# centreborelli/sat-bundleadjust

Measured on AMD Instinct MI355X. Metric: LM iters/sec at 200 cams x 1M pts x 10M obs (affine, R+T), higher is better.
Workload: dtype f64; 1 GPU; C4: 200 cams x 1000000 pts x 9998866 obs, affine, correction R+T, 1 fixed camera, seed 1; obs_per_rank0=9998866

## Files before the change

sat-bundleadjust_amd/csrc/satba_capi.hip:

```cpp
#include <hip/hip_runtime.h>

#include <algorithm>
#include <atomic>
#include <chrono>
#include <cmath>
#include <cstdarg>
#include <cstdio>
#include <cstdlib>
#include <cstring>
#include <new>
#include <string>
#include <thread>
#include <vector>

#include "../../include/satba.h"
#include "satba_chol.h"
#include "satba_kernels.h"
#include "satba_layout.h"
#include "satba_lm.h"
#include "satba_lmdev.h"
#include "satba_outliers.h"
#include "satba_triangulate.h"
#include "satba_tracks.h"
#include "satba_ftracks.h"
// ... 48 lines not shown
        if (e_ != hipSuccess) return fail(SATBA_E_HIP, "%s: %s (%s:%d)", #expr, hipGetErrorString(e_), __FILE__, __LINE__); \
    } while (0)

constexpr int RED_SLOTS = 8, RED_MAX_GRID = 2048, RED_MAX_NV = 4;
struct SchurItems { int2* items = nullptr; SchurItem* desc = nullptr; int n_blocks = 0; };
static_assert(sizeof(SchurItemKey) == sizeof(int2) && offsetof(SchurItemKey, pair) == offsetof(int2, x) && offsetof(SchurItemKey, chunk) == offsetof(int2, y), "uploaded as int2");

struct satba_problem {
    int model = 0, M = 0, N = 0, NP = 0, c_p = 0, n_cam_fix = 0, n_pts_fix = 0, rank = 0, world = 1, f32 = 0, device = 0;
    long long K = 0, n_total = 0;
    int n_c = 0, n = 0, hdr = 0;
    int loss = 0;
    int camc_lds = 0, rpc_lds = 0;
    int cam_sums_lds = 1;
    int lin_rep_shift = 0;
    int deterministic = 0;
    int split_env = -1;
    double *d_fx = nullptr, *d_bbox = nullptr, *d_fxcost = nullptr, *d_fxcost_new = nullptr, *d_fxcost0 = nullptr;
    int *d_fxflag = nullptr, *d_fxe = nullptr;
    bool fxcost_valid = false, fxcost_new_valid = false, fxcost0_valid = false;
    double w_max = 1.0, n_max_cam = 1.0, fx_shrink = 1.0;
    int fx_fallbacks = 0;
    bool scales_by_tail = false;
    bool prep_fused = false;
    struct LmDev* d_lm = nullptr;
    struct LmSummary* h_lm = nullptr;
    struct LmSummary* h_lm_dev = nullptr;
    long long lm_ticks_queued = 0;
    hipStream_t own_stream = nullptr;
    double f_scale = 1.0, lead = 1.0;
    hipStream_t stream = nullptr;
    Layout L;
    int unit_weights = 0;
    double *d_cam_static = nullptr, *d_rpc = nullptr;
    double *d_x = nullptr, *d_xnew = nullptr, *d_camc = nullptr, *d_camc_new = nullptr;
    double *d_scale_inv = nullptr, *d_g = nullptr, *d_gh = nullptr, *d_gn = nullptr, *d_q1 = nullptr, *d_wv = nullptr;
    double *d_U = nullptr, *d_gc = nullptr, *d_V = nullptr, *d_PV = nullptr, *d_dc = nullptr, *d_dch = nullptr;
    double2 *d_f = nullptr, *d_ftmp = nullptr;
    bool f_valid = false;
    bool prof_lin = false;
    std::vector<hipEvent_t> prof_ev;
    size_t prof_used = 0;
    double* d_Jpm = nullptr;
    double *d_part = nullptr, *d_part3 = nullptr, *d_pair_part = nullptr;
    SchurItems items_chunked;
    SchurItems items_merged;
// ... 205 lines not shown
    if (unit_run(p))
        SATBA_DISPATCH(p, hipLaunchKernelGGL((k_residual<MODEL, NP, CL, RL, true, false>), dim3(grid), dim3(RES_THREADS), lds, p->stream, a, f, p->red(RB_RES), cost, t));
    else
        SATBA_DISPATCH(p, hipLaunchKernelGGL((k_residual<MODEL, NP, CL, RL, false, false>), dim3(grid), dim3(RES_THREADS), lds, p->stream, a, f, p->red(RB_RES), cost, t));
    HIP_TRY(hipGetLastError());
    return 0;
}

static int launch_trial(satba_problem* p, const PhaseCtx& c, double c0, double c1, const double* v0, const double* v1) {
    if (c.decide1a_in_trial) {
        hipLaunchKernelGGL(k_lm_decide1a_trial_cams, dim3(1), dim3(256), 0, p->stream, p->d_lm, p->d_xb, p->model, p->M, p->NP, p->c_p, p->d_x, v0, v1,
                           p->d_scale_inv, p->d_cam_static, p->d_xnew, p->d_camc_new, p->d_xb, (int)p->hdr);
    } else
    hipLaunchKernelGGL(k_trial_cams, dim3((std::max(p->M, (int)p->hdr) + 63) / 64), dim3(64), 0, p->stream, p->model, p->M, p->NP, p->c_p, p->d_x, v0, v1,
                       p->d_scale_inv, c0, c1, p->d_cam_static, p->d_xnew, p->d_camc_new, p->d_xb, (int)p->hdr, c.coef_dev, c.gate);
    HIP_TRY(hipGetLastError());
    ObsArgs a = obs_args(p, true, c.gate);
    a.sh = slice_split(p);
    a.rev = slice_rev(3);
    const int grid = slice_grid(p, RES_THREADS / 64, 2, a.sh);
    const size_t lds = table_bytes(p);
    TrialArgs t{p->d_x, v0, v1, p->d_scale_inv, p->d_xnew, c0, c1, p->lead, p->d_xb + SATBA_HDR_STEP_SQ, p->d_xb + SATBA_HDR_X_SQ, p->d_fxcost_new, c.coef_dev};
    if (c.decide2_in_trial) { t.lm_st = p->d_lm; t.lm_sum = p->h_lm_dev; }
    p->fxcost_new_valid = true;
    double* cost = p->d_xb + SATBA_HDR_COST_NEW;
    if (unit_run(p))
        SATBA_DISPATCH(p, hipLaunchKernelGGL((k_residual<MODEL, NP, CL, RL, true, true>), dim3(grid), dim3(RES_THREADS), lds, p->stream, a, (double2*)nullptr, p->red(RB_RES), cost, t));
    else
        SATBA_DISPATCH(p, hipLaunchKernelGGL((k_residual<MODEL, NP, CL, RL, false, true>), dim3(grid), dim3(RES_THREADS), lds, p->stream, a, (double2*)nullptr, p->red(RB_RES), cost, t));
    HIP_TRY(hipGetLastError());
    return 0;
}

static int lin_variant(const satba_problem* p) {
    if (p->loss == 0) return (p->unit_weights && p->model != RPC) ? 0 : 1;
    return p->loss == SATBA_LOSS_SOFT_L1 ? 2 : 3;
}

template <int MODEL, int NP, bool CL, bool RL>
static int launch_lin(satba_problem* p, const ObsArgs& a) {
    double* gpv = p->d_g + p->n_c;
    double* cost = p->d_xb + SATBA_HDR_COST;
    double* gmax = p->d_xb + SATBA_HDR_FIXED + p->rank;
    const size_t lds = lin_lds(p);
    const RedBuf rb = p->red(RB_LIN);
    constexpr bool BIGL = MODEL == RPC || NP > 6;
// ... 23 lines not shown
    TRY(raise_lds_limit(k_linearize<MODEL, NP, false, CL, RL, false, false, true>, lds));
    TRY(raise_lds_limit(k_linearize<MODEL, NP, false, CL, RL, false, false, false>, lds));
    TRY(raise_lds_limit(k_linearize<MODEL, NP, true, CL, RL, false, false, true>, lds));
    TRY(raise_lds_limit(k_linearize<MODEL, NP, true, CL, RL, false, false, false>, lds));
    TRY(raise_lds_limit(k_linearize<MODEL, NP, true, CL, RL, true, false, true>, lds));
    TRY(raise_lds_limit(k_linearize<MODEL, NP, true, CL, RL, true, false, false>, lds));
    if constexpr (MODEL != RPC) {
        TRY(raise_lds_limit(k_linearize<MODEL, NP, false, CL, RL, false, true, true>, lds));
        TRY(raise_lds_limit(k_linearize<MODEL, NP, false, CL, RL, false, true, false>, lds));
    }
    TRY(raise_lds_limit(k_residual<MODEL, NP, CL, RL, true, false>, table_bytes(p)));
    TRY(raise_lds_limit(k_residual<MODEL, NP, CL, RL, false, false>, table_bytes(p)));
    TRY(raise_lds_limit(k_residual<MODEL, NP, CL, RL, true, true>, table_bytes(p)));
    TRY(raise_lds_limit(k_residual<MODEL, NP, CL, RL, false, true>, table_bytes(p)));
    const size_t dirb = p->dir_global ? 0 : dir_table_bytes(p);
    const size_t t = std::max(table_bytes(p), dirb);
    TRY(raise_lds_limit(k_jvp<MODEL, NP, 1, CL, RL, true>, t));
    TRY(raise_lds_limit(k_jvp<MODEL, NP, 1, CL, RL, false>, t));
    TRY(raise_lds_limit(k_jvp<MODEL, NP, 2, CL, RL, false>, std::max(t, 2 * dirb)));
    TRY(raise_lds_limit(k_backsub<MODEL, NP, CL, RL>, t));
    return 0;
}

static int launch_linearize_kernel(satba_problem* p, const PhaseCtx& c) {
    ObsArgs a = obs_args(p, false, c.gate);
    a.sh = slice_split(p);
    a.rev = slice_rev(0);
    if (c.fuse_prep >= 0) {
        a.prep_scale = p->d_scale_inv; a.prep_gh = p->d_gh; a.prep_ghs = p->d_q1;
        a.prep_first = c.fuse_prep; a.prep_first_dev = c.first_dev;
    }
    const bool prof = p->prof_lin && p->prof_used + 2 <= 2 * 4096;
    if (prof) {
        while (p->prof_ev.size() < p->prof_used + 2) {
            hipEvent_t e;
            HIP_TRY(hipEventCreate(&e));
            p->prof_ev.push_back(e);
        }
        HIP_TRY(hipEventRecord(p->prof_ev[p->prof_used], p->stream));
    }
    SATBA_DISPATCH(p, TRY((launch_lin<MODEL, NP, CL, RL>(p, a))));
    if (prof) {
        HIP_TRY(hipEventRecord(p->prof_ev[p->prof_used + 1], p->stream));
        p->prof_used += 2;
    }
    return 0;
}

static int launch_cam_sums(satba_problem* p, const int* gate, double* U, double* gc) {
    ObsArgs a = obs_args(p, false, gate);
    CamMajor cm = cam_major(p);
    SATBA_DISPATCH(p, hipLaunchKernelGGL((k_cam_sums<MODEL, NP>), dim3(p->M, p->cm_chunks), dim3(LINC_THREADS), 0, p->stream, a, cm, p->d_f, p->d_part3));
// ... 8 lines not shown
struct SchurRoute;
int schur_items_build(satba_problem* p, SchurTable kind, SchurItems* t, long long dg_weight);
int schur_item_tables(satba_problem* p);
template <int MODEL, int NP> int launch_schur(satba_problem* p, const FrontCtx& f, const SchurRoute& r, const ObsArgs& a, double* S, double* rhs);
}
static int launch_schur_kernel(satba_problem* p, const int* gate, const FrontCtx& f, const SchurRoute& r) {
    ObsArgs a = obs_args(p, false, gate);
    double* S = p->payload();
    double* rhs = S + (size_t)p->n_c * p->n_c;
    SATBA_DISPATCH(p, TRY((launch_schur<MODEL, NP>(p, f, r, a, S, rhs))));
    return 0;
}

static int launch_backsub_kernel(satba_problem* p, const int* gate) {
    ObsArgs a = obs_args(p, false, gate);
    a.sh = slice_split(p);
    a.rev = slice_rev(1);
    const int grid = slice_grid(p, BS_THREADS / 64, 2, a.sh);
    const size_t lds = p->model == AFFINE ? dir_table_bytes(p) : table_bytes(p);
    if (p->dir_global) {
        SATBA_DISPATCH(p, if constexpr (MODEL == AFFINE) {
            hipLaunchKernelGGL((k_affine_dir_tab<NP>), dim3(1), dim3(1024), 0, p->stream, a, p->d_dc, (const double*)nullptr, (const double*)nullptr);
            hipLaunchKernelGGL((k_backsub<MODEL, NP, CL, RL, true>), dim3(grid), dim3(BS_THREADS), 0, p->stream, a, p->d_dc, p->d_dch, p->lead,
                               p->d_V, p->d_lam_used, p->d_g, p->d_scale_inv, p->d_gh, p->d_gn, p->red(RB_BS), p->d_xb);
        });
    } else
    SATBA_DISPATCH(p, hipLaunchKernelGGL((k_backsub<MODEL, NP, CL, RL>), dim3(grid), dim3(BS_THREADS), lds, p->stream, a, p->d_dc, p->d_dch, p->lead,
                                         p->d_V, p->d_lam_used, p->d_g, p->d_scale_inv, p->d_gh, p->d_gn, p->red(RB_BS), p->d_xb));
    HIP_TRY(hipGetLastError());
    return 0;
}

static int launch_jvp(satba_problem* p, const int* gate, int nv, const double* q1, const double* q2, double* out, bool pre = false) {
    ObsArgs a = obs_args(p, false, gate);
    a.sh = slice_split(p);
    a.rev = slice_rev(2);
    const int grid = slice_grid(p, JVP_THREADS / 64, 2, a.sh);
    const RedBuf rb = p->red(RB_JVP);
    if (p->dir_global && (nv == 2 || pre)) {
        SATBA_DISPATCH(p, if constexpr (MODEL == AFFINE) {
            hipLaunchKernelGGL((k_affine_dir_tab<NP>), dim3(1), dim3(1024), 0, p->stream, a, q1, nv == 2 ? q2 : nullptr, nv == 2 ? p->d_scale_inv : nullptr);
            if (nv == 1) hipLaunchKernelGGL((k_jvp<MODEL, NP, 1, CL, RL, true, true>), dim3(grid), dim3(JVP_THREADS), 0, p->stream, a, q1, q2, p->d_scale_inv, rb, out);
            else hipLaunchKernelGGL((k_jvp<MODEL, NP, 2, CL, RL, false, true>), dim3(grid), dim3(JVP_THREADS), 0, p->stream, a, q1, q2, p->d_scale_inv, rb, out);
        });
    } else if (nv == 1 && pre) {
        const size_t lds = p->model == AFFINE ? dir_table_bytes(p) : table_bytes(p);
        SATBA_DISPATCH(p, hipLaunchKernelGGL((k_jvp<MODEL, NP, 1, CL, RL, true>), dim3(grid), dim3(JVP_THREADS), lds, p->stream, a, q1, q2, p->d_scale_inv, rb, out));
    } else if (nv == 1) {
        SATBA_DISPATCH(p, hipLaunchKernelGGL((k_jvp<MODEL, NP, 1, CL, RL, false>), dim3(grid), dim3(JVP_THREADS), table_bytes(p), p->stream, a, q1, q2,
                                             p->d_scale_inv, rb, out));
    } else {
        const size_t lds = p->model == AFFINE ? std::max(table_bytes(p), 2 * dir_table_bytes(p)) : table_bytes(p);
        SATBA_DISPATCH(p, hipLaunchKernelGGL((k_jvp<MODEL, NP, 2, CL, RL, false>), dim3(grid), dim3(JVP_THREADS), lds, p->stream, a, q1, q2,
                                             p->d_scale_inv, rb, out));
    }
    HIP_TRY(hipGetLastError());
    return 0;
}

static int dense_solve(satba_problem* p, const int* gate, double* S, double* b, bool cleared = false, bool* unscaled = nullptr) {
    TrsvTail tail;
    tail.dc = p->d_dc; tail.scale_inv = p->d_scale_inv; tail.hdr = p->d_xb; tail.hdr_len = (int)p->hdr; tail.fail = p->d_fail; tail.lead = p->lead;
    tail.keep = p->d_keep; tail.keep_at = SATBA_HDR_KEEP; tail.keep_len = SATBA_KEEP_LEN;
    const bool done = cholesky_solve(S, p->n_c, b, p->d_fail, p->d_fail + 1, p->stream, p->chol, p->d_dinv, cleared, gate, nullptr,
                                     unscaled ? &tail : nullptr);
    if (unscaled) *unscaled = done;
    HIP_TRY(hipGetLastError());
    return 0;
}

__global__ void k_lambda(const double* __restrict__ hdr, double Delta, double lam_floor, double* __restrict__ keep, const double* __restrict__ Delta_dev,
                         const double* __restrict__ lam_force, const int* gate) {
    SATBA_GATE(gate);
    if (Delta_dev) Delta = *Delta_dev;
    if (lam_force && *lam_force > 0.0) { keep[SATBA_KEEP_LAM] = *lam_force; return; }
    (void)schur_lambda(hdr, Delta, lam_floor, keep, true);
}
// ... 660 lines not shown
    }
    HIP_TRY(hipStreamSynchronize(p->stream));
    if (host_cost) *host_cost = p->h_pin[0];
    return 0;
}

static int linearize_impl(satba_problem* p, const PhaseCtx& c) {
    Range range_("satba:linearize");
    TRY(ensure_wlayout(p));
    const size_t nU = (size_t)p->M * p->NP * p->NP;
    const int n_clear = (int)(p->hdr + nU + p->n_c);
    if (p->cam_sums_lds) {
        if (p->loss == 0 && !p->fxcost_valid) {
            TRY(launch_residual(p, false, nullptr, p->d_fxcost, c.gate));
            p->fxcost_valid = true;
        }
        if (!c.skip_lin_scales)
        SATBA_DISPATCH(p, hipLaunchKernelGGL((k_lin_scales<MODEL, NP>), dim3(1), dim3(256), 0, p->stream, p->M, p->d_camc, p->d_rpc, p->d_bbox, p->w_max,
                                             p->loss, p->f_scale, p->d_fxcost, p->n_max_cam, p->fx_shrink, p->d_fx, p->d_fxe, p->d_fxflag, p->d_xb, n_clear, c.gate));
        HIP_TRY(hipGetLastError());
    } else {
        HIP_TRY(hipMemsetAsync(p->d_xb, 0, sizeof(double) * n_clear, p->stream));
    }
    TRY(launch_linearize_kernel(p, c));
    double* U = p->payload();
    double* gc = U + nU;
    if (p->cam_sums_lds) {
        const int const_t = lin_const_t(p->model, p->NP, p->loss != 0, unit_run(p)) && lin_variant(p) == 0;
        const int total = p->M * 2 * p->NP;
        hipLaunchKernelGGL(k_lin_finish, dim3((total + 63) / 64), dim3(1024), 0, p->stream, p->M, p->NP, p->lin_grid, p->d_part, U, gc,
                           p->L.cam_ofs, p->d_camc, p->n_cam_fix, const_t, p->d_fx, p->d_fxe, p->d_fxflag, p->d_xb + SATBA_HDR_FX, c.gate);
        HIP_TRY(hipGetLastError());
    } else {
        TRY(launch_cam_sums(p, c.gate, U, gc));
    }
    p->linearized = true; p->have_step = false;
    p->f_valid = !p->cam_sums_lds && p->model == RPC;
    p->prep_fused = c.fuse_prep >= 0;
    return 0;
}
int satba_linearize(satba_problem* p) {
    if (!p) return fail(SATBA_E_ARG, "null handle");
    HIP_TRY(hipSetDevice(p->device));
    return linearize_impl(p, PhaseCtx{});
}

static int prepare_impl(satba_problem* p, const PhaseCtx& c, int first) {
    Range range_("satba:prepare");
    if (!p->linearized) return fail(SATBA_E_STATE, "prepare before linearize");
    const size_t nU = (size_t)p->M * p->NP * p->NP;
    if (p->hdr > 1024) return fail(SATBA_E_ARG, "header too long");
    if (p->prep_fused && p->n_c <= 1024) {
        hipLaunchKernelGGL(k_prepare_cams, dim3(1), dim3(1024), 0, p->stream, (int)nU, p->n_c, p->NP, p->world, SATBA_HDR_FIXED, (int)p->hdr, first, p->lead,
                           p->d_xb, p->d_U, p->d_gc, p->d_keep, p->d_x, p->d_g, p->d_scale_inv, p->d_gh, p->d_q1, c.first_dev, c.gate);
        HIP_TRY(hipGetLastError());
        TRY(launch_jvp(p, c.gate, 1, p->d_q1, p->d_q1, p->d_xb + SATBA_HDR_JG_SQ, true));
        p->prepared = true;
        return 0;
    }
    hipLaunchKernelGGL(k_prepare_stash, dim3(1), dim3(1024), 0, p->stream, (int)nU, p->n_c, p->world, SATBA_HDR_FIXED, (int)p->hdr, p->d_xb, p->d_U,
                       p->d_gc, p->d_keep, c.gate);
    HIP_TRY(hipGetLastError());
    const int n_prep = p->prep_fused ? p->n_c : p->n;
    hipLaunchKernelGGL(k_prepare_vec, dim3(grid_for(n_prep, 256, 1024)),
                       dim3(256), 0, p->stream, n_prep, p->n_c, p->NP, first,
                       p->lead, p->d_U, p->d_gc, p->d_V, p->d_x, p->d_g, p->d_scale_inv, p->d_gh, p->d_q1, p->red(RB_PREP), p->d_xb, p->d_keep, c.first_dev, c.gate);
    HIP_TRY(hipGetLastError());
    TRY(launch_jvp(p, c.gate, 1, p->d_q1, p->d_q1, p->d_xb + SATBA_HDR_JG_SQ, true));
    p->prepared = true;
    return 0;
}
int satba_prepare(satba_problem* p, int32_t first) {
    if (!p) return fail(SATBA_E_ARG, "null handle");
    HIP_TRY(hipSetDevice(p->device));
    return prepare_impl(p, PhaseCtx{}, first);
}

static int solve_impl(satba_problem* p, const PhaseCtx& c);
#include "satba_schur_api.inc"
// ... 17 lines not shown
    bool unscaled = false;
    TRY(dense_solve(p, c.gate, S, p->d_dch, true, &unscaled));
    if (!unscaled) {
        const int nu = std::max(p->n_c, (int)p->hdr);
        hipLaunchKernelGGL(k_unscale, dim3((nu + 255) / 256), dim3(256), 0, p->stream, p->n_c, p->d_scale_inv, p->d_dch, p->d_dc, (int)p->hdr,
                           p->d_xb, p->d_fail, p->lead, p->d_keep, SATBA_HDR_KEEP, SATBA_KEEP_LEN, c.gate);
        HIP_TRY(hipGetLastError());
    }
    TRY(launch_backsub_kernel(p, c.gate));
    p->have_step = true;
    return 0;
}
int satba_solve(satba_problem* p) {
    if (!p) return fail(SATBA_E_ARG, "null handle");
    HIP_TRY(hipSetDevice(p->device));
    return solve_impl(p, PhaseCtx{});
}

static int subspace_impl(satba_problem* p, const PhaseCtx& c, double alpha, double inv_norm_g) {
    Range range_("satba:subspace");
    if (!p->have_step) return fail(SATBA_E_STATE, "subspace before solve");
    if (!c.gate) TRY(zero_header(p));
    hipLaunchKernelGGL(k_subspace_vec, dim3(grid_for(p->n, 256, 512)), dim3(256), 0, p->stream, p->n, p->n_c, p->lead, alpha,
                       inv_norm_g, p->d_gh, p->d_gn, p->d_q1, p->d_wv, p->red(RB_SUB), p->d_xb, c.sub_args_dev, c.gate);
    HIP_TRY(hipGetLastError());
    return 0;
}
int satba_subspace(satba_problem* p, double alpha, double inv_norm_g) {
    if (!p) return fail(SATBA_E_ARG, "null handle");
    HIP_TRY(hipSetDevice(p->device));
    return subspace_impl(p, PhaseCtx{}, alpha, inv_norm_g);
}

static int subspace_products_impl(satba_problem* p, const PhaseCtx& c) {
    Range range_("satba:subspace_products");
    if (!p->have_step) return fail(SATBA_E_STATE, "subspace_products before solve");
    if (!c.gate) TRY(zero_header(p));
    return launch_jvp(p, c.gate, 2, p->d_q1, p->d_wv, p->d_xb + SATBA_HDR_B11);
}
int satba_subspace_products(satba_problem* p) {
    if (!p) return fail(SATBA_E_ARG, "null handle");
    HIP_TRY(hipSetDevice(p->device));
    return subspace_products_impl(p, PhaseCtx{});
}

static int trial_impl(satba_problem* p, const PhaseCtx& c, bool gn, double c0, double c1) {
    Range range_("satba:trial");
    if (!p->have_step) return fail(SATBA_E_STATE, "trial before solve");
// ... 112 lines not shown
}

int satba_profile_read(satba_problem* p, int64_t* n_launches, double* ms_total) {
    if (!p || !n_launches || !ms_total) return fail(SATBA_E_ARG, "null argument");
    HIP_TRY(hipSetDevice(p->device));
    HIP_TRY(hipStreamSynchronize(p->stream));
    double tot = 0.0;
    for (size_t i = 0; i + 1 < p->prof_used; i += 2) {
        float ms = 0.f;
        HIP_TRY(hipEventElapsedTime(&ms, p->prof_ev[i], p->prof_ev[i + 1]));
        tot += ms;
    }
    *n_launches = (int64_t)(p->prof_used / 2);
    *ms_total = tot;
    p->prof_used = 0;
    return 0;
}

int satba_get_vector(satba_problem* p, int32_t which, double* host_out) {
    if (!p || !host_out) return fail(SATBA_E_ARG, "null argument");
    const double* src[] = {p->d_g, p->d_scale_inv, p->d_gn, p->d_q1, p->d_wv, p->d_xnew, p->d_gh};
    if (which < 0 || which > 6) return fail(SATBA_E_ARG, "unknown vector id %d", which);
    HIP_TRY(hipSetDevice(p->device));
    return download_permuted(p, src[which], host_out, p->n_c, 3);
}

int64_t satba_layout_len(const satba_problem* p, int32_t which) {
    if (!p) return -1;
    const Layout& L = p->L;
    switch (which) {
        case SATBA_LAY_PERM: case SATBA_LAY_RANK: case SATBA_LAY_PT_CNT: return L.N;
        case SATBA_LAY_SLICE_BASE: return L.n_slices + 1;
        case SATBA_LAY_E_CAM: return L.P;
        case SATBA_LAY_OBS_POS: case SATBA_LAY_CM_PT: case SATBA_LAY_CM_POS: case SATBA_LAY_CM_IO: return L.K;
        case SATBA_LAY_IPT_OFS: return L.N + 1;
        case SATBA_LAY_CAM_OFS: return L.M + 1;
        case SATBA_LAY_PAIR_OFS: return L.n_pairs * (L.C + 1) + 1;
        case SATBA_LAY_PAIR_PTS: case SATBA_LAY_PAIR_PI: case SATBA_LAY_PAIR_PJ: return L.E;
        case SATBA_LAY_PAIR_IJ: return 2 * L.n_pairs;
        case SATBA_LAY_W_FIX: case SATBA_LAY_SC_OFS: return L.wl_ready ? L.N + 1 : -1;
        case SATBA_LAY_PAIR_REC: case SATBA_LAY_PAIR_KK: return L.wl_ready ? L.E : -1;
        case SATBA_LAY_CM_REC: case SATBA_LAY_CM_SC: return L.wl_ready ? L.K : -1;
        case SATBA_LAY_DG_OFS: return L.wl_ready ? (long long)L.M * L.n_dg + 1 : -1;
        default: return -1;
    }
}
// ... 44 lines not shown
    out[5] = p->L.P; out[6] = (double)p->L.E; out[7] = p->L.C; out[8] = p->unit_weights; out[9] = p->camc_lds; out[10] = p->rpc_lds;
    out[11] = p->cam_sums_lds; out[12] = p->deterministic; out[13] = p->cm_chunks; out[14] = p->lin_grid; out[15] = p->fx_fallbacks;
    if (n > 16) out[16] = (lm_device_loop_ok(p) && lm_device_loop_pays(p)) ? 1.0 : 0.0;
    if (n > 17) out[17] = p->beside_off ? -1.0 : (p->beside_last ? 1.0 : 0.0);
    if (n > 18) out[18] = p->beside_timeouts;
    if (n > 19) out[19] = p->L.wl_ready ? p->L.dg_spc : 0;
    if (n > 20) out[20] = slice_split(p);
    if (n > 21) out[21] = p->lin_rep_shift;
    return 0;
}

int satba_time_kernel(satba_problem* p, int32_t phase, int32_t reps, float* ms_avg) {
    if (!p || !ms_avg || reps <= 0) return fail(SATBA_E_ARG, "bad argument");
    if (phase < 0 || phase > 5) return fail(SATBA_E_ARG, "unknown phase %d", phase);
    if (phase >= 2 && !p->linearized) return fail(SATBA_E_STATE, "time_kernel: linearize first");
    HIP_TRY(hipSetDevice(p->device));
    hipEvent_t e0, e1;
    HIP_TRY(hipEventCreate(&e0));
    HIP_TRY(hipEventCreate(&e1));
    int rc = 0;
    auto once = [&]() -> int {
        switch (phase) {
            case 0: return launch_residual(p, false, p->d_f, p->d_scal);
            case 1: return launch_linearize_kernel(p, PhaseCtx{});
            case 2: return launch_schur_kernel(p, nullptr, FrontCtx{}, schur_route(p, FrontCtx{}));
            case 3: {
                return dense_solve(p, nullptr, p->payload(), p->d_dch);
            }
            case 4: return launch_backsub_kernel(p, nullptr);
            default: return launch_jvp(p, nullptr, 1, p->d_q1, p->d_q1, p->d_scal, true);
        }
    };
    rc = once();
    if (!rc) {
        (void)hipEventRecord(e0, p->stream);
        for (int i = 0; i < reps && !rc; ++i) rc = once();
        (void)hipEventRecord(e1, p->stream);
        (void)hipEventSynchronize(e1);
        float ms = 0.f;
        (void)hipEventElapsedTime(&ms, e0, e1);
        *ms_avg = ms / reps;
    }
    (void)hipEventDestroy(e0);
    (void)hipEventDestroy(e1);
    p->linearized = false; p->have_step = false;
    return rc;
}
// ... 11 lines not shown
```

sat-bundleadjust_amd/csrc/satba_kernels.h:

```cpp
#pragma once
#include <hip/hip_runtime.h>
#include <stdint.h>

#include "../../include/satba.h"
#include "satba_models.h"

namespace satba {

__host__ __device__ constexpr int cam_acc_len(int np) { return np * (np + 1) / 2 + np; }
__host__ __device__ constexpr int cam_acc_stride(int np) { return cam_acc_len(np) | 1; }
__host__ __device__ constexpr int cam_sum_len(int np) { return 3 * np; }
__host__ __device__ constexpr int cam_sum_stride(int np) { return (3 * np) | 1; }
constexpr int FX_LO_SHIFT = 40;
constexpr long long FX_MAX_OBS_PER_CAM = 1ll << 23;
__host__ __device__ constexpr size_t cam_sum_bytes(int np, size_t rows) { return (rows * cam_sum_stride(np) * 8 + 15) & ~(size_t)15; }
__host__ __device__ constexpr int fx_scales_len(int np) { return 2 * np; }
__host__ __device__ constexpr int fx_exps_len(int np) { return np + 3; }

constexpr int RPCS = 94;
static_assert(RPCS >= 90 && RPCS % 2 == 0 && (RPCS / 2) % 2 == 1, "RPC rows in the LDS: an odd number of 16-byte slots");
constexpr double FX_MAGIC = 6755399441055744.0;
constexpr unsigned long long FX_MAGIC_BITS = 0x4338000000000000ull;
__host__ __device__ constexpr int jrow_stride(int) { return 8; }

// ... 292 lines not shown
                              double* __restrict__ out, int dir) {
    const long long total = (long long)n_c + (long long)N * dim;
    for (long long i = (long long)blockIdx.x * blockDim.x + threadIdx.x; i < total; i += (long long)gridDim.x * blockDim.x) {
        if (i < n_c) { out[i] = in[i]; continue; }
        const long long j = i - n_c;
        const int q = (int)(j / dim), k = (int)(j % dim);
        const long long ext = (long long)n_c + (long long)perm[q] * dim + k;
        if (dir == 0) out[i] = in[ext];
        else out[ext] = in[i];
    }
}
__global__ void k_gather_obs(long long K, const int* __restrict__ obs_pos, const double2* __restrict__ f, double2* __restrict__ out) {
    for (long long o = (long long)blockIdx.x * blockDim.x + threadIdx.x; o < K; o += (long long)gridDim.x * blockDim.x) out[o] = f[obs_pos[o]];
}

__global__ void k_gather_obs1(long long K, const int* __restrict__ obs_pos, const double* __restrict__ v, double* __restrict__ out) {
    for (long long o = (long long)blockIdx.x * blockDim.x + threadIdx.x; o < K; o += (long long)gridDim.x * blockDim.x) out[o] = v[obs_pos[o]];
}

#ifndef SATBA_RES_THREADS
#define SATBA_RES_THREADS 512
#endif
constexpr int RES_THREADS = SATBA_RES_THREADS;
struct TrialArgs {
    const double* __restrict__ x;
    const double* __restrict__ v0;
    const double* __restrict__ v1;
    const double* __restrict__ scale_inv;
    double* __restrict__ x_new;
    double c0, c1, lead;
    double* ss;
    double* xx;
    double* cost2;
    const double* coef;
    struct LmDev* lm_st = nullptr;
    struct LmSummary* lm_sum = nullptr;
};
__device__ void lm_decide2_body(struct LmDev* gst, double cost_new, double step_sq, double x_sq, struct LmSummary* sum);
template <int MODEL, int NP, bool CL, bool RL, bool UNITW = false, bool TRIAL = false>
__global__ __launch_bounds__(RES_THREADS) void k_residual(ObsArgs a, double2* __restrict__ f, RedBuf rb, double* __restrict__ cost, TrialArgs t) {
    if (a.gate != nullptr && *a.gate == 0) {
        if constexpr (TRIAL) {
            if (t.lm_st && blockIdx.x == 0 && threadIdx.x == 0) lm_decide2_body(t.lm_st, 0.0, 0.0, 0.0, t.lm_sum);
        }
        return;
    }
    if constexpr (TRIAL) { if (t.coef) { t.c0 = t.coef[0]; t.c1 = t.coef[1]; } }
    extern __shared__ __attribute__((aligned(16))) double s_dyn_res[];
    CamTables<CL, RL> T;
    T.stage(a, s_dyn_res, RES_THREADS);
    const int lane = threadIdx.x & 63;
    constexpr int WAVES = RES_THREADS / 64;
    double acc = 0.0, ss = 0.0, xx = 0.0;
    if (TRIAL && blockIdx.x == 0) {
        for (int i = threadIdx.x; i < a.n_c; i += RES_THREADS) {
            const double step = (t.c0 * t.v0[i] + t.c1 * t.v1[i]) / t.scale_inv[i], xi = t.x[i];
            ss += t.lead * step * step; xx += t.lead * xi * xi;
        }
    }
    for_each_slice(a.n_slices << a.sh, WAVES, [&](const int u) {
        const SliceUnit su(a, u, lane);
        const int q = su.q;
        const bool has = q < a.N;
        const int cnt = has ? a.pt_cnt[q] : 0;
        double X = 0.0, Y = 0.0, Z = 0.0;
        if (has) {
            const size_t ip = (size_t)a.n_c + 3 * (size_t)q;
            if constexpr (TRIAL) {
                double xn[3];
#pragma unroll
                for (int k = 0; k < 3; ++k) {
                    const double step = (t.c0 * t.v0[ip + k] + t.c1 * t.v1[ip + k]) / t.scale_inv[ip + k], xi = t.x[ip + k];
                    xn[k] = xi + step;
                    if (su.g == 0) { t.x_new[ip + k] = xn[k]; ss += step * step; xx += xi * xi; }
                }
                X = xn[0]; Y = xn[1]; Z = xn[2];
            } else {
                const double* px = a.x + ip; X = px[0]; Y = px[1]; Z = px[2];
            }
        }
        int pos = su.pos;
        ObsRec r[SATBA_PF + 1];
#pragma unroll
        for (int j = 0; j < SATBA_PF; ++j) r[j].template load<UNITW>(a, pos + su.step * j, su.slot(j) < cnt);
        for (int tt = 0; tt < su.nt; ++tt, pos += su.step) {
            const int k = su.slot(tt);
            r[SATBA_PF].load<UNITW>(a, pos + su.step * SATBA_PF, su.slot(tt + SATBA_PF) < cnt);
            __builtin_amdgcn_sched_barrier(0);
            if (k < cnt) {
                ObsEval<MODEL, NP, false, !UNITW, false, UNITW> e;
                e.eval(a, r[0].cam, 1.0, T.cc(r[0].cam), T.tab(r[0].cam), r[0].ob, r[0].w, X, Y, Z);
                if (f) f[pos] = make_double2(e.ftrue[0], e.ftrue[1]);
                acc += e.rho;
            }
#pragma unroll
// ... 135 lines not shown
#pragma unroll
            for (int k = 0; k < 9; ++k) v[k] = slice_point_sum(v[k], su.sh);
        }
        if (has && su.g == 0) {
            if constexpr (UNITW) {
#pragma unroll
                for (int k = 0; k < 9; ++k) v[k] *= mp;
            }
            double2* vo = reinterpret_cast<double2*>(V + 6 * (size_t)q);
            vo[0] = make_double2(v[0], v[1]); vo[1] = make_double2(v[2], v[3]); vo[2] = make_double2(v[4], v[5]);
            double* go = gp + 3 * (size_t)q;
            go[0] = v[6]; go[1] = v[7]; go[2] = v[8];
            gmax = fmax(gmax, fmax(fabs(v[6]), fmax(fabs(v[7]), fabs(v[8]))));
            if (a.prep_scale) {
                const size_t ib = (size_t)a.n_c + 3 * (size_t)q;
                const double dg[3] = {v[0], v[3], v[5]}, xv[3] = {X, Y, Z};
#pragma unroll
                for (int k = 0; k < 3; ++k) {
                    double si = sqrt(dg[k]);
                    if (prep_first) si = (si == 0.0) ? 1.0 : si;
                    else si = fmax(si, a.prep_scale[ib + k]);
                    a.prep_scale[ib + k] = si;
                    const double h = v[6 + k] / si;
                    a.prep_gh[ib + k] = h;
                    a.prep_ghs[ib + k] = h / si;
                    s_gh += h * h;
                    const double xs = xv[k] * si;
                    s_xs += xs * xs;
                }
            }
        }
    }, a.rev);
    gmax = wave_max(gmax);
    if (lane == 0 && gmax > 0.0) atomic_max_pos(hdr_gpmax, gmax);
    if constexpr (CAMSUMS) {
        if (bad != 0ull && lane == 0) atomicOr(a.fx_flag, 1);
#ifdef SATBA_ABLATE_CAM_ATOMICS
        if (abl == 0x5a5a5a5a5a5a5a5aull) atomicOr(a.fx_flag, 4);
#endif
        __syncthreads();
        unsigned long long* out = reinterpret_cast<unsigned long long*>(part) + (size_t)blockIdx.x * a.M * 3 * NP;
        for (int i = threadIdx.x; i < a.M * 3 * NP; i += THREADS) {
            const int cam = i / (3 * NP), k = i % (3 * NP);
            unsigned long long t = 0ull;
            for (int r = 0; r < (1 << a.rep_shift); ++r) t += s_acc[(size_t)((cam << a.rep_shift) | r) * CUS + k];
            out[i] = t;
        }
    }
// ... 366 lines not shown
            for (int i = 0; i < 3; ++i) k[i] = vs ? vc[c * NP + 5 + i] * (1.0 / vs[c * NP + 5 + i]) : vc[c * NP + 5 + i];
#pragma unroll
            for (int m = 0; m < 3; ++m) { B[0][m] += k[0] * cc[6 + m] + k[2] * cc[9 + m]; B[1][m] += k[1] * cc[9 + m]; }
            b[0] += k[0] * cc[CAMX] + k[2] * cc[CAMX + 1];
            b[1] += k[1] * cc[CAMX + 1];
        }
        double* row = tab + (size_t)c * JVP_ROW;
#pragma unroll
        for (int m = 0; m < 3; ++m) { row[m] = mc * B[0][m]; row[3 + m] = mc * B[1][m]; row[8 + m] = Jp[0][m]; row[11 + m] = Jp[1][m]; }
        row[6] = mc * b[0]; row[7] = mc * b[1];
    }
    __syncthreads();
}

template <int NP>
__global__ __launch_bounds__(1024) void k_affine_dir_tab(ObsArgs a, const double* __restrict__ v1, const double* __restrict__ v2, const double* __restrict__ vs) {
    SATBA_GATE(a.gate);
    affine_dir_table<NP>(a, v1, a.dir_tab, 1024, vs);
    if (v2) affine_dir_table<NP>(a, v2, a.dir_tab + (size_t)a.M * JVP_ROW, 1024, vs);
}

template <int MODEL, int NP, int NV, bool CL, bool RL, bool PRE, bool DG = false>
__global__ __launch_bounds__(JVP_THREADS) void k_jvp(ObsArgs a, const double* __restrict__ q1, const double* __restrict__ q2,
                                                     const double* __restrict__ scale_inv, RedBuf rb, double* __restrict__ out) {
    SATBA_GATE(a.gate);
    extern __shared__ __attribute__((aligned(16))) double s_dyn_jvp[];
    const int lane = threadIdx.x & 63;
    constexpr int WAVES = JVP_THREADS / 64;
    double s11 = 0.0, s12 = 0.0, s22 = 0.0;
    if constexpr (MODEL == AFFINE && PRE && NV == 1) {
        const double* tab = DG ? a.dir_tab : s_dyn_jvp;
        if constexpr (!DG) affine_dir_table<NP>(a, q1, s_dyn_jvp, JVP_THREADS);
        for_each_slice(a.n_slices << a.sh, WAVES, [&](const int u) {
            const SliceUnit su(a, u, lane);
            const int q = su.q;
            const bool has = q < a.N;
            const int cnt = has ? a.pt_cnt[q] : 0;
            double X = 0.0, Y = 0.0, Z = 0.0, v0 = 0.0, v1 = 0.0, v2 = 0.0;
            if (has) {
                const size_t ip = (size_t)a.n_c + 3 * (size_t)q;
                X = a.x[ip]; Y = a.x[ip + 1]; Z = a.x[ip + 2];
                const double mp = (a.perm[q] >= a.n_pts_fix) ? 1.0 : 0.0;
                v0 = mp * q1[ip]; v1 = mp * q1[ip + 1]; v2 = mp * q1[ip + 2];
            }
            int pos = su.pos;
            const int io0 = has ? a.ipt_ofs[q] : 0;
            constexpr int D = SATBA_CAM_PF;
            int cq[D];
            double2 sq[D];
#pragma unroll
            for (int d = 0; d < D; ++d) {
                const int kd = su.slot(d);
                cq[d] = 0; sq[d] = make_double2(1.0, 1.0);
                if (kd < cnt) { cq[d] = a.e_cam[pos + d * su.step]; if (a.sc) sq[d] = a.sc[io0 + kd]; }
            }
            for (int tt = 0; tt < su.nt; ++tt, pos += su.step) {
                const int k = su.slot(tt), kn = su.slot(tt + D);
                int cn = 0;
                double2 sn = make_double2(1.0, 1.0);
                if (kn < cnt) { cn = a.e_cam[pos + D * su.step]; if (a.sc) sn = a.sc[io0 + kn]; }
                __builtin_amdgcn_sched_barrier(0);
                const int c0 = cq[0];
                const double2 s0 = sq[0];
                if (k < cnt) {
                    DirRow R;
                    R.load(tab, c0);
// ... 64 lines not shown
                    s12 += u0 * w0 + u1 * w1;
                    s22 += w0 * w0 + w1 * w1;
                }
#pragma unroll
                for (int d = 0; d + 1 < D; ++d) { cq[d] = cq[d + 1]; sq[d] = sq[d + 1]; }
                cq[D - 1] = cn; sq[D - 1] = sn;
            }
        }, a.rev);
    } else {
        CamTables<CL, RL> T;
        T.stage(a, s_dyn_jvp, JVP_THREADS);
        for_each_slice(a.n_slices << a.sh, WAVES, [&](const int u) {
            const SliceUnit su(a, u, lane);
            const int q = su.q;
            const bool has = q < a.N;
            const int cnt = has ? a.pt_cnt[q] : 0;
            double X = 0.0, Y = 0.0, Z = 0.0, mp = 0.0, p1[3] = {0, 0, 0}, p2[3] = {0, 0, 0};
            if (has) {
                const size_t ip = (size_t)a.n_c + 3 * (size_t)q;
                X = a.x[ip]; Y = a.x[ip + 1]; Z = a.x[ip + 2];
                mp = (a.perm[q] >= a.n_pts_fix) ? 1.0 : 0.0;
#pragma unroll
                for (int j = 0; j < 3; ++j) {
                    if constexpr (PRE) p1[j] = q1[ip + j];
                    else {
                        const double si = 1.0 / scale_inv[ip + j];
                        p1[j] = q1[ip + j] * si;
                        if (NV == 2) p2[j] = q2[ip + j] * si;
                    }
                }
            }
            int pos = su.pos;
            const int io0 = has ? a.ipt_ofs[q] : 0;
            for (int tt = 0; tt < su.nt; ++tt, pos += su.step) {
                const int k = su.slot(tt);
                if (k < cnt) {
                    const int cam = a.e_cam[pos];
                    ObsEval<MODEL, NP, true> e;
                    e.jac(a, io0 + k, cam, mp, T.cc(cam), T.tab(cam), X, Y, Z);
                    const size_t ic = (size_t)cam * NP;
                    double j1[2] = {0, 0}, j2[2] = {0, 0};
#pragma unroll
                    for (int i = 0; i < NP; ++i) {
                        double v1;
                        if constexpr (PRE) v1 = q1[ic + i];
                        else {
                            const double si = 1.0 / scale_inv[ic + i];
// ... 141 lines not shown
        xb[SATBA_HDR_XS_SQ] = b + s_k[1];
        xb[SATBA_HDR_GC_INF] = lead * m;
    }
}

__device__ __forceinline__ void point_block_inverse(double v0, double v1, double v2, double v3, double v4, double v5, double lam, double s0,
                                                    double s1, double s2, double (&o)[6]) {
    const double a = v0 + lam * s0 * s0, b = v1, c = v2;
    const double d = v3 + lam * s1 * s1, e = v4, f = v5 + lam * s2 * s2;
    const double c00 = d * f - e * e, c01 = c * e - b * f, c02 = b * e - c * d;
    const double idet = 1.0 / (a * c00 + b * c01 + c * c02);
    o[0] = c00 * idet; o[1] = c01 * idet; o[2] = c02 * idet;
    o[3] = (a * f - c * c) * idet; o[4] = (b * c - a * e) * idet; o[5] = (a * d - b * b) * idet;
}

#ifndef SATBA_BS_THREADS
#define SATBA_BS_THREADS 512
#endif
constexpr int BS_THREADS = SATBA_BS_THREADS;
template <int MODEL, int NP, bool CL, bool RL, bool DG = false>
__global__ __launch_bounds__(BS_THREADS) void k_backsub(ObsArgs a, const double* __restrict__ dc, const double* __restrict__ dch,
                                                        double lead, const double* __restrict__ V, const double* __restrict__ lam_used,
                                                        const double* __restrict__ g, const double* __restrict__ scale_inv, const double* __restrict__ gh,
                                                        double* __restrict__ gn, RedBuf rb, double* __restrict__ hdr) {
    SATBA_GATE(a.gate);
    extern __shared__ __attribute__((aligned(16))) double s_dyn_bs[];
    const int lane = threadIdx.x & 63;
    constexpr int WAVES = BS_THREADS / 64;
    double sa = 0.0, sb = 0.0, sc = 0.0;
    if (blockIdx.x == 0) {
        for (int i = threadIdx.x; i < a.n_c; i += BS_THREADS) {
            const double v = dch[i], h = gh[i];
            gn[i] = v;
            sa += lead * h * h; sb += lead * h * v; sc += lead * v * v;
        }
    }
    CamTables<CL, RL> T;
    const double* tab = DG ? a.dir_tab : s_dyn_bs;
    if constexpr (MODEL == AFFINE) { if constexpr (!DG) affine_dir_table<NP>(a, dc, s_dyn_bs, BS_THREADS); }
    else T.stage(a, s_dyn_bs, BS_THREADS);
    for_each_slice(a.n_slices << a.sh, WAVES, [&](const int u) {
        const SliceUnit su(a, u, lane);
        const int q = su.q;
        const bool has = q < a.N;
        const int cnt = has ? a.pt_cnt[q] : 0;
        double X = 0.0, Y = 0.0, Z = 0.0, mp = 0.0;
        if (has) {
// ... 49 lines not shown
                        u0 += e.Jc[0][i] * d;
                        u1 += e.Jc[1][i] * d;
                    }
#pragma unroll
                    for (int j = 0; j < 3; ++j) t[j] += e.Jp[0][j] * u0 + e.Jp[1][j] * u1;
                }
            }
        }
        if (su.sh) {
#pragma unroll
            for (int j = 0; j < 3; ++j) t[j] = slice_point_sum(t[j], su.sh);
        }
        if (has && su.g == 0) {
            const size_t ib = (size_t)a.n_c + 3 * (size_t)q;
            const double2* v2 = reinterpret_cast<const double2*>(V + 6 * (size_t)q);
            const double2 va = v2[0], vb = v2[1], vc = v2[2];
            double vi[6];
            point_block_inverse(va.x, va.y, vb.x, vb.y, vc.x, vc.y, *lam_used, scale_inv[ib], scale_inv[ib + 1], scale_inv[ib + 2], vi);
            const double r0 = g[ib] - t[0], r1 = g[ib + 1] - t[1], r2 = g[ib + 2] - t[2];
            const double d[3] = {vi[0] * r0 + vi[1] * r1 + vi[2] * r2, vi[1] * r0 + vi[3] * r1 + vi[4] * r2,
                                 vi[2] * r0 + vi[4] * r1 + vi[5] * r2};
#pragma unroll
            for (int k = 0; k < 3; ++k) {
                const double v = d[k] * scale_inv[ib + k], h = gh[ib + k];
                gn[ib + k] = v;
                sa += h * h; sb += h * v; sc += v * v;
            }
        }
    }, a.rev);
    double v[3] = {sa, sb, sc};
    double* const dst[3] = {hdr + SATBA_HDR_GRAM_A, hdr + SATBA_HDR_GRAM_B, hdr + SATBA_HDR_GRAM_C};
    grid_sum<3>(v, dst, rb);
}

__global__ __launch_bounds__(256) void k_subspace_vec(int n, int n_c, double lead, double alpha, double s,
                                                      const double* __restrict__ gh, const double* __restrict__ gn,
                                                      double* __restrict__ q1, double* __restrict__ wv, RedBuf rb,
                                                      double* __restrict__ hdr, const double* __restrict__ args_dev, const int* gate) {
    SATBA_GATE(gate);
    if (args_dev) { alpha = args_dev[0]; s = args_dev[1]; }
    double ww = 0.0, wq = 0.0, gw = 0.0;
    for (int i = blockIdx.x * blockDim.x + threadIdx.x; i < n; i += gridDim.x * blockDim.x) {
        const double h = gh[i], q = s * h, w = gn[i] - alpha * h;
        q1[i] = q;
        wv[i] = w;
        const double wgt = (i < n_c) ? lead : 1.0;
        ww += wgt * w * w; wq += wgt * w * q; gw += wgt * h * w;
    }
    double v[3] = {ww, wq, gw};
    double* const dst[3] = {hdr + SATBA_HDR_WW, hdr + SATBA_HDR_WQ1, hdr + SATBA_HDR_GHW};
    grid_sum<3>(v, dst, rb);
}

template <int MODEL, int NP>
__global__ void k_jacobian(ObsArgs a, const int* __restrict__ pts_ind, const int* __restrict__ rank, const int* __restrict__ obs_pos,
                           double* __restrict__ Jc, double* __restrict__ Jp) {
    for (long long o = (long long)blockIdx.x * blockDim.x + threadIdx.x; o < a.K; o += (long long)gridDim.x * blockDim.x) {
        const int p = pts_ind[o], q = rank[p], pos = obs_pos[o], cam = a.e_cam[pos];
        const double* px = a.x + a.n_c + 3 * (size_t)q;
        ObsEval<MODEL, NP, true> e;
        e.eval(a, cam, (p >= a.n_pts_fix) ? 1.0 : 0.0, a.camc + (size_t)cam * CAMC, (MODEL == RPC) ? a.rpc + (size_t)cam * 90 : nullptr,
               a.e_obs[pos], a.e_w[pos], px[0], px[1], px[2]);
        for (int r = 0; r < 2; ++r) {
            for (int i = 0; i < NP; ++i) Jc[(o * 2 + r) * NP + i] = e.Jc[r][i];
            for (int j = 0; j < 3; ++j) Jp[(o * 2 + r) * 3 + j] = e.Jp[r][j];
        }
    }
}

}
```

Before: 907.5 LM iters/sec.

## Recompute point scaled gradient on the fly instead of storing gh/ghs arrays

Skips writing the point portions of the scaled gradient (gh) and its doubly scaled copy (q1) during the fused linearize prep. The consumers (trial, jvp precondition, backsub, subspace) instead recompute them from g and scale_inv. A fill kernel materialises them lazily when the host downloads those vectors. This cuts two 3M-double writes per linearize and swaps some reads for division work, at the cost of state-tracking flags and more reader complexity.

```diff
diff --git a/sat-bundleadjust_amd/csrc/satba_capi.hip b/sat-bundleadjust_amd/csrc/satba_capi.hip
--- a/sat-bundleadjust_amd/csrc/satba_capi.hip
+++ b/sat-bundleadjust_amd/csrc/satba_capi.hip
@@ -94,6 +94,8 @@
     double w_max = 1.0, n_max_cam = 1.0, fx_shrink = 1.0;
     int fx_fallbacks = 0;
     bool scales_by_tail = false;
+    bool gh_in_readers = false;
+    bool q1_points_unformed = false;
     bool prep_fused = false;
     struct LmDev* d_lm = nullptr;
     struct LmSummary* h_lm = nullptr;
@@ -345,6 +347,7 @@
     const size_t lds = table_bytes(p);
     TrialArgs t{p->d_x, v0, v1, p->d_scale_inv, p->d_xnew, c0, c1, p->lead, p->d_xb + SATBA_HDR_STEP_SQ, p->d_xb + SATBA_HDR_X_SQ, p->d_fxcost_new, c.coef_dev};
     if (c.decide2_in_trial) { t.lm_st = p->d_lm; t.lm_sum = p->h_lm_dev; }
+    if (v0 == p->d_gh && p->gh_in_readers) t.g_pts = p->d_g;
     p->fxcost_new_valid = true;
     double* cost = p->d_xb + SATBA_HDR_COST_NEW;
     if (unit_run(p))
@@ -414,12 +417,19 @@
     return 0;
 }
 
-static int launch_linearize_kernel(satba_problem* p, const PhaseCtx& c) {
+static bool points_gh_stored(const satba_problem* p, const PhaseCtx& c) {
+    const char* e = getenv("SATBA_STORE_GH");
+    const bool off = e && atoi(e) != 0;
+    return off || !(c.fuse_prep >= 0 && p->world == 1 && p->n_c <= 1024 && p->cam_sums_lds);
+}
+
+static int launch_linearize_kernel(satba_problem* p, const PhaseCtx& c, bool store_gh) {
     ObsArgs a = obs_args(p, false, c.gate);
     a.sh = slice_split(p);
     a.rev = slice_rev(0);
     if (c.fuse_prep >= 0) {
-        a.prep_scale = p->d_scale_inv; a.prep_gh = p->d_gh; a.prep_ghs = p->d_q1;
+        a.prep_scale = p->d_scale_inv;
+        if (store_gh) { a.prep_gh = p->d_gh; a.prep_ghs = p->d_q1; }
         a.prep_first = c.fuse_prep; a.prep_first_dev = c.first_dev;
     }
     const bool prof = p->prof_lin && p->prof_used + 2 <= 2 * 4096;
@@ -474,11 +484,11 @@
         SATBA_DISPATCH(p, if constexpr (MODEL == AFFINE) {
             hipLaunchKernelGGL((k_affine_dir_tab<NP>), dim3(1), dim3(1024), 0, p->stream, a, p->d_dc, (const double*)nullptr, (const double*)nullptr);
             hipLaunchKernelGGL((k_backsub<MODEL, NP, CL, RL, true>), dim3(grid), dim3(BS_THREADS), 0, p->stream, a, p->d_dc, p->d_dch, p->lead,
-                               p->d_V, p->d_lam_used, p->d_g, p->d_scale_inv, p->d_gh, p->d_gn, p->red(RB_BS), p->d_xb);
+                               p->d_V, p->d_lam_used, p->d_g, p->d_scale_inv, p->d_gh, p->d_gn, p->red(RB_BS), p->d_xb, p->gh_in_readers ? nullptr : p->d_gh);
         });
     } else
     SATBA_DISPATCH(p, hipLaunchKernelGGL((k_backsub<MODEL, NP, CL, RL>), dim3(grid), dim3(BS_THREADS), lds, p->stream, a, p->d_dc, p->d_dch, p->lead,
-                                         p->d_V, p->d_lam_used, p->d_g, p->d_scale_inv, p->d_gh, p->d_gn, p->red(RB_BS), p->d_xb));
+                                         p->d_V, p->d_lam_used, p->d_g, p->d_scale_inv, p->d_gh, p->d_gn, p->red(RB_BS), p->d_xb, p->gh_in_readers ? nullptr : p->d_gh));
     HIP_TRY(hipGetLastError());
     return 0;
 }
@@ -489,22 +499,23 @@
     a.rev = slice_rev(2);
     const int grid = slice_grid(p, JVP_THREADS / 64, 2, a.sh);
     const RedBuf rb = p->red(RB_JVP);
+    const double* g_pre = (pre && p->gh_in_readers) ? p->d_g : nullptr;
     if (p->dir_global && (nv == 2 || pre)) {
         SATBA_DISPATCH(p, if constexpr (MODEL == AFFINE) {
             hipLaunchKernelGGL((k_affine_dir_tab<NP>), dim3(1), dim3(1024), 0, p->stream, a, q1, nv == 2 ? q2 : nullptr, nv == 2 ? p->d_scale_inv : nullptr);
-            if (nv == 1) hipLaunchKernelGGL((k_jvp<MODEL, NP, 1, CL, RL, true, true>), dim3(grid), dim3(JVP_THREADS), 0, p->stream, a, q1, q2, p->d_scale_inv, rb, out);
-            else hipLaunchKernelGGL((k_jvp<MODEL, NP, 2, CL, RL, false, true>), dim3(grid), dim3(JVP_THREADS), 0, p->stream, a, q1, q2, p->d_scale_inv, rb, out);
+            if (nv == 1) hipLaunchKernelGGL((k_jvp<MODEL, NP, 1, CL, RL, true, true>), dim3(grid), dim3(JVP_THREADS), 0, p->stream, a, q1, q2, p->d_scale_inv, rb, out, g_pre);
+            else hipLaunchKernelGGL((k_jvp<MODEL, NP, 2, CL, RL, false, true>), dim3(grid), dim3(JVP_THREADS), 0, p->stream, a, q1, q2, p->d_scale_inv, rb, out, g_pre);
         });
     } else if (nv == 1 && pre) {
         const size_t lds = p->model == AFFINE ? dir_table_bytes(p) : table_bytes(p);
-        SATBA_DISPATCH(p, hipLaunchKernelGGL((k_jvp<MODEL, NP, 1, CL, RL, true>), dim3(grid), dim3(JVP_THREADS), lds, p->stream, a, q1, q2, p->d_scale_inv, rb, out));
+        SATBA_DISPATCH(p, hipLaunchKernelGGL((k_jvp<MODEL, NP, 1, CL, RL, true>), dim3(grid), dim3(JVP_THREADS), lds, p->stream, a, q1, q2, p->d_scale_inv, rb, out, g_pre));
     } else if (nv == 1) {
         SATBA_DISPATCH(p, hipLaunchKernelGGL((k_jvp<MODEL, NP, 1, CL, RL, false>), dim3(grid), dim3(JVP_THREADS), table_bytes(p), p->stream, a, q1, q2,
-                                             p->d_scale_inv, rb, out));
+                                             p->d_scale_inv, rb, out, g_pre));
     } else {
         const size_t lds = p->model == AFFINE ? std::max(table_bytes(p), 2 * dir_table_bytes(p)) : table_bytes(p);
         SATBA_DISPATCH(p, hipLaunchKernelGGL((k_jvp<MODEL, NP, 2, CL, RL, false>), dim3(grid), dim3(JVP_THREADS), lds, p->stream, a, q1, q2,
-                                             p->d_scale_inv, rb, out));
+                                             p->d_scale_inv, rb, out, g_pre));
     }
     HIP_TRY(hipGetLastError());
     return 0;
@@ -1211,7 +1222,8 @@
     } else {
         HIP_TRY(hipMemsetAsync(p->d_xb, 0, sizeof(double) * n_clear, p->stream));
     }
-    TRY(launch_linearize_kernel(p, c));
+    const bool store_gh = points_gh_stored(p, c);
+    TRY(launch_linearize_kernel(p, c, store_gh));
     double* U = p->payload();
     double* gc = U + nU;
     if (p->cam_sums_lds) {
@@ -1226,6 +1238,8 @@
     p->linearized = true; p->have_step = false;
     p->f_valid = !p->cam_sums_lds && p->model == RPC;
     p->prep_fused = c.fuse_prep >= 0;
+    p->gh_in_readers = !store_gh;
+    p->q1_points_unformed = false;
     return 0;
 }
 int satba_linearize(satba_problem* p) {
@@ -1244,6 +1258,7 @@
                            p->d_xb, p->d_U, p->d_gc, p->d_keep, p->d_x, p->d_g, p->d_scale_inv, p->d_gh, p->d_q1, c.first_dev, c.gate);
         HIP_TRY(hipGetLastError());
         TRY(launch_jvp(p, c.gate, 1, p->d_q1, p->d_q1, p->d_xb + SATBA_HDR_JG_SQ, true));
+        p->q1_points_unformed = p->gh_in_readers;
         p->prepared = true;
         return 0;
     }
@@ -1307,8 +1322,10 @@
     if (!p->have_step) return fail(SATBA_E_STATE, "subspace before solve");
     if (!c.gate) TRY(zero_header(p));
     hipLaunchKernelGGL(k_subspace_vec, dim3(grid_for(p->n, 256, 512)), dim3(256), 0, p->stream, p->n, p->n_c, p->lead, alpha,
-                       inv_norm_g, p->d_gh, p->d_gn, p->d_q1, p->d_wv, p->red(RB_SUB), p->d_xb, c.sub_args_dev, c.gate);
-    HIP_TRY(hipGetLastError());
+                       inv_norm_g, p->d_gh, p->d_gn, p->d_q1, p->d_wv, p->red(RB_SUB), p->d_xb, c.sub_args_dev, c.gate,
+                       p->gh_in_readers ? p->d_g : nullptr, p->d_scale_inv);
+    HIP_TRY(hipGetLastError());
+    p->q1_points_unformed = false;
     return 0;
 }
 int satba_subspace(satba_problem* p, double alpha, double inv_norm_g) {
@@ -1467,6 +1484,13 @@
     const double* src[] = {p->d_g, p->d_scale_inv, p->d_gn, p->d_q1, p->d_wv, p->d_xnew, p->d_gh};
     if (which < 0 || which > 6) return fail(SATBA_E_ARG, "unknown vector id %d", which);
     HIP_TRY(hipSetDevice(p->device));
+    const bool fill_gh = which == 6 && p->gh_in_readers, fill_q1 = which == 3 && p->gh_in_readers && p->q1_points_unformed;
+    if (fill_gh || fill_q1) {
+        hipLaunchKernelGGL(k_fill_point_gh, dim3(grid_for(p->n - p->n_c, 256, 1024)), dim3(256), 0, p->stream, (long long)p->n_c, (long long)p->n, p->d_g,
+                           p->d_scale_inv, fill_gh ? p->d_gh : (double*)nullptr, fill_q1 ? p->d_q1 : (double*)nullptr);
+        if (fill_q1) p->q1_points_unformed = false;
+        HIP_TRY(hipGetLastError());
+    }
     return download_permuted(p, src[which], host_out, p->n_c, 3);
 }
 
@@ -1557,7 +1581,7 @@
     auto once = [&]() -> int {
         switch (phase) {
             case 0: return launch_residual(p, false, p->d_f, p->d_scal);
-            case 1: return launch_linearize_kernel(p, PhaseCtx{});
+            case 1: return launch_linearize_kernel(p, PhaseCtx{}, true);
             case 2: return launch_schur_kernel(p, nullptr, FrontCtx{}, schur_route(p, FrontCtx{}));
             case 3: {
                 return dense_solve(p, nullptr, p->payload(), p->d_dch);
diff --git a/sat-bundleadjust_amd/csrc/satba_kernels.h b/sat-bundleadjust_amd/csrc/satba_kernels.h
--- a/sat-bundleadjust_amd/csrc/satba_kernels.h
+++ b/sat-bundleadjust_amd/csrc/satba_kernels.h
@@ -338,6 +338,12 @@
 #define SATBA_RES_THREADS 512
 #endif
 constexpr int RES_THREADS = SATBA_RES_THREADS;
+__device__ inline double point_gh(const double* __restrict__ g, const double* __restrict__ scale_inv, size_t i) { return g[i] / scale_inv[i]; }
+__device__ inline double point_ghs(const double* __restrict__ g, const double* __restrict__ scale_inv, size_t i) {
+    const double si = scale_inv[i];
+    return (g[i] / si) / si;
+}
+
 struct TrialArgs {
     const double* __restrict__ x;
     const double* __restrict__ v0;
@@ -351,6 +357,7 @@
     const double* coef;
     struct LmDev* lm_st = nullptr;
     struct LmSummary* lm_sum = nullptr;
+    const double* __restrict__ g_pts = nullptr;
 };
 __device__ void lm_decide2_body(struct LmDev* gst, double cost_new, double step_sq, double x_sq, struct LmSummary* sum);
 template <int MODEL, int NP, bool CL, bool RL, bool UNITW = false, bool TRIAL = false>
@@ -386,7 +393,8 @@
                 double xn[3];
 #pragma unroll
                 for (int k = 0; k < 3; ++k) {
-                    const double step = (t.c0 * t.v0[ip + k] + t.c1 * t.v1[ip + k]) / t.scale_inv[ip + k], xi = t.x[ip + k];
+                    const double v0k = t.g_pts ? point_gh(t.g_pts, t.scale_inv, ip + k) : t.v0[ip + k];
+                    const double step = (t.c0 * v0k + t.c1 * t.v1[ip + k]) / t.scale_inv[ip + k], xi = t.x[ip + k];
                     xn[k] = xi + step;
                     if (su.g == 0) { t.x_new[ip + k] = xn[k]; ss += step * step; xx += xi * xi; }
                 }
@@ -568,8 +576,10 @@
                     else si = fmax(si, a.prep_scale[ib + k]);
                     a.prep_scale[ib + k] = si;
                     const double h = v[6 + k] / si;
-                    a.prep_gh[ib + k] = h;
-                    a.prep_ghs[ib + k] = h / si;
+                    if (a.prep_gh) {
+                        a.prep_gh[ib + k] = h;
+                        a.prep_ghs[ib + k] = h / si;
+                    }
                     s_gh += h * h;
                     const double xs = xv[k] * si;
                     s_xs += xs * xs;
@@ -982,7 +992,8 @@
 
 template <int MODEL, int NP, int NV, bool CL, bool RL, bool PRE, bool DG = false>
 __global__ __launch_bounds__(JVP_THREADS) void k_jvp(ObsArgs a, const double* __restrict__ q1, const double* __restrict__ q2,
-                                                     const double* __restrict__ scale_inv, RedBuf rb, double* __restrict__ out) {
+                                                     const double* __restrict__ scale_inv, RedBuf rb, double* __restrict__ out,
+                                                     const double* __restrict__ g_pre) {
     SATBA_GATE(a.gate);
     extern __shared__ __attribute__((aligned(16))) double s_dyn_jvp[];
     const int lane = threadIdx.x & 63;
@@ -1001,7 +1012,8 @@
                 const size_t ip = (size_t)a.n_c + 3 * (size_t)q;
                 X = a.x[ip]; Y = a.x[ip + 1]; Z = a.x[ip + 2];
                 const double mp = (a.perm[q] >= a.n_pts_fix) ? 1.0 : 0.0;
-                v0 = mp * q1[ip]; v1 = mp * q1[ip + 1]; v2 = mp * q1[ip + 2];
+                if (g_pre) { v0 = mp * point_ghs(g_pre, scale_inv, ip); v1 = mp * point_ghs(g_pre, scale_inv, ip + 1); v2 = mp * point_ghs(g_pre, scale_inv, ip + 2); }
+                else { v0 = mp * q1[ip]; v1 = mp * q1[ip + 1]; v2 = mp * q1[ip + 2]; }
             }
             int pos = su.pos;
             const int io0 = has ? a.ipt_ofs[q] : 0;
@@ -1112,7 +1124,7 @@
                 mp = (a.perm[q] >= a.n_pts_fix) ? 1.0 : 0.0;
 #pragma unroll
                 for (int j = 0; j < 3; ++j) {
-                    if constexpr (PRE) p1[j] = q1[ip + j];
+                    if constexpr (PRE) p1[j] = g_pre ? point_ghs(g_pre, scale_inv, ip + j) : q1[ip + j];
                     else {
                         const double si = 1.0 / scale_inv[ip + j];
                         p1[j] = q1[ip + j] * si;
@@ -1300,7 +1312,7 @@
 __global__ __launch_bounds__(BS_THREADS) void k_backsub(ObsArgs a, const double* __restrict__ dc, const double* __restrict__ dch,
                                                         double lead, const double* __restrict__ V, const double* __restrict__ lam_used,
                                                         const double* __restrict__ g, const double* __restrict__ scale_inv, const double* __restrict__ gh,
-                                                        double* __restrict__ gn, RedBuf rb, double* __restrict__ hdr) {
+                                                        double* __restrict__ gn, RedBuf rb, double* __restrict__ hdr, const double* __restrict__ gh_pts) {
     SATBA_GATE(a.gate);
     extern __shared__ __attribute__((aligned(16))) double s_dyn_bs[];
     const int lane = threadIdx.x & 63;
@@ -1396,7 +1408,7 @@
                                  vi[2] * r0 + vi[4] * r1 + vi[5] * r2};
 #pragma unroll
             for (int k = 0; k < 3; ++k) {
-                const double v = d[k] * scale_inv[ib + k], h = gh[ib + k];
+                const double v = d[k] * scale_inv[ib + k], h = gh_pts ? gh_pts[ib + k] : point_gh(g, scale_inv, ib + k);
                 gn[ib + k] = v;
                 sa += h * h; sb += h * v; sc += v * v;
             }
@@ -1410,12 +1422,13 @@
 __global__ __launch_bounds__(256) void k_subspace_vec(int n, int n_c, double lead, double alpha, double s,
                                                       const double* __restrict__ gh, const double* __restrict__ gn,
                                                       double* __restrict__ q1, double* __restrict__ wv, RedBuf rb,
-                                                      double* __restrict__ hdr, const double* __restrict__ args_dev, const int* gate) {
+                                                      double* __restrict__ hdr, const double* __restrict__ args_dev, const int* gate,
+                                                      const double* __restrict__ g_pts, const double* __restrict__ scale_inv) {
     SATBA_GATE(gate);
     if (args_dev) { alpha = args_dev[0]; s = args_dev[1]; }
     double ww = 0.0, wq = 0.0, gw = 0.0;
     for (int i = blockIdx.x * blockDim.x + threadIdx.x; i < n; i += gridDim.x * blockDim.x) {
-        const double h = gh[i], q = s * h, w = gn[i] - alpha * h;
+        const double h = (g_pts && i >= n_c) ? point_gh(g_pts, scale_inv, (size_t)i) : gh[i], q = s * h, w = gn[i] - alpha * h;
         q1[i] = q;
         wv[i] = w;
         const double wgt = (i < n_c) ? lead : 1.0;
@@ -1426,6 +1439,13 @@
     grid_sum<3>(v, dst, rb);
 }
 
+__global__ __launch_bounds__(256) void k_fill_point_gh(long long n_c, long long n, const double* __restrict__ g, const double* __restrict__ scale_inv,
+                                                       double* __restrict__ gh, double* __restrict__ ghs) {
+    for (long long i = n_c + (long long)blockIdx.x * blockDim.x + threadIdx.x; i < n; i += (long long)gridDim.x * blockDim.x) {
+        if (gh) gh[i] = point_gh(g, scale_inv, (size_t)i);
+        if (ghs) ghs[i] = point_ghs(g, scale_inv, (size_t)i);
+    }
+}
 template <int MODEL, int NP>
 __global__ void k_jacobian(ObsArgs a, const int* __restrict__ pts_ind, const int* __restrict__ rank, const int* __restrict__ obs_pos,
                            double* __restrict__ Jc, double* __restrict__ Jp) {
```

Result: faster. 918.4 LM iters/sec, median of 6 (+1.2%).
